# JanEGerken/HEAL-SWIN

Hardware: AMD Instinct MI355X
Metric: images/sec fwd+bwd, HEAL-SWIN nside=256 seg, batch=8 at 1/2/4/8 MI355X (higher is better)
Workload: dtype bf16

## Files before the change

### heal_swin_amd/_lib.py

```python
import ctypes
import os

import numpy as np

_PKG = os.path.dirname(os.path.abspath(__file__))
LIB_PATH = os.path.join(_PKG, "lib", "libhealswin.so")

HS_F32, HS_BF16 = 0, 1
HS_F64 = 3
HS_PRED_LABELS, HS_PRED_ROWS16 = 2, 4
HS_ATTN_COSINE = 1
HS_ATTN_FORCE_VALU = 2
HS_ATTN_RESIDUAL = 4
HS_ATTN_OVERWRITE_GRADS = 8
HS_EPI_BIAS, HS_EPI_GELU, HS_EPI_DGELU, HS_EPI_RESID = 0, 1, 2, 3
HS_ACC_DEFER = 2
HS_MLP_NORM_AFTER = 16
HS_U8, HS_I32, HS_I64 = 8, 9, 10
HS_FLAT_PATCH_ROWS, HS_FLAT_PIXEL_ROWS = 0, 1
HS_DEPTH_L1, HS_DEPTH_L2, HS_DEPTH_HUBER, HS_DEPTH_LOGVAR = 0, 1, 2, 3
HS_DT_NONE, HS_DT_LOG, HS_DT_INV = 0, 1, 2
HS_DT_ZERO_BKG, HS_DT_1000_BKG, HS_DT_AFFINE, HS_DT_INVERSE = 1, 2, 4, 8
HS_DEPTH_STATS_WORDS = 15

c_i64 = ctypes.c_int64
c_int = ctypes.c_int
c_uint = ctypes.c_uint
c_ptr = ctypes.c_void_p
c_float = ctypes.c_float

_SIGNATURES = {
    "hs_nest2ring": [c_int, c_ptr, c_ptr, c_i64],
    "hs_ring2nest": [c_int, c_ptr, c_ptr, c_i64],
    "hs_nest_win_idcs": [c_int, c_ptr],
    "hs_rel_pos_index": [c_int, c_ptr],
    "hs_build_nest_roll_shift": [c_i64, c_int, c_int, c_ptr, c_ptr, c_ptr],
    "hs_build_nest_grid_shift": [c_int, c_int, c_int, c_ptr, c_ptr, c_ptr],
    "hs_build_ring_shift": [c_int, c_int, c_int, c_int, c_ptr, c_ptr, c_ptr],
    "hs_attn_mask_from_labels": [c_ptr, c_i64, c_int, c_ptr],
    "hs_flat_zorder": [c_int, c_int, c_int, c_ptr, c_ptr],
    "hs_build_flat_shift": [c_int, c_int, c_int, c_int, c_int, c_ptr, c_ptr, c_ptr],
    "hs_flat_rel_pos_index": [c_int, c_ptr, c_ptr],
    "hs_flat_attn_mask": [c_int, c_int, c_int, c_int, c_ptr],
    "hs_flat_img_to_rows": [c_ptr, c_int, c_ptr, c_int, c_int, c_int, c_int, c_int, c_int, c_int, c_int, c_i64, c_ptr],
    "hs_flat_rows_to_img": [c_ptr, c_int, c_ptr, c_int, c_int, c_int, c_int, c_int, c_int, c_int, c_int, c_i64, c_ptr],
    "hs_rel_bias_gather": [c_ptr, c_ptr, c_ptr, c_int, c_int, c_int, c_ptr],
    "hs_rel_bias_scatter_grad_sorted_add": [c_ptr, c_ptr, c_ptr, c_ptr, c_int, c_int, c_int, c_ptr],
    "hs_cos_head_scale_fwd": [c_ptr, c_ptr, c_int, c_ptr],
    "hs_cos_head_scale_bwd": [c_ptr, c_ptr, c_ptr, c_int, c_int, c_ptr],
    "hs_rel_bias_gather_many": [c_ptr, c_ptr, c_int, c_ptr, c_ptr, c_int, c_int, c_ptr],
    "hs_rel_bias_scatter_grad_sorted_many": [c_ptr, c_ptr, c_ptr, c_ptr, c_int, c_ptr, c_ptr, c_int, c_int, c_ptr],
    "hs_cos_head_scale_many": [c_ptr, c_ptr, c_ptr, c_ptr, c_ptr, c_int, c_ptr],
# ... 23 lines not shown
    "hs_backproject_labels": [c_ptr, c_int, c_i64, c_i64, c_int, c_i64, c_i64, c_i64, c_ptr, c_i64, c_int, c_ptr, c_ptr],
    "hs_backproject_image": [c_ptr, c_i64, c_i64, c_ptr, c_ptr, c_i64, c_ptr, c_ptr],
    "hs_seg_confusion": [c_ptr, c_int, c_i64, c_i64, c_int, c_i64, c_i64, c_i64, c_ptr, c_i64, c_ptr, c_int, c_ptr, c_ptr, c_ptr],
    "hs_depth_points": [c_ptr, c_int, c_i64, c_i64, c_i64, c_i64, c_i64, c_i64, c_ptr, c_i64, c_ptr, c_int, c_ptr, c_ptr, c_ptr, c_ptr,
                        c_ptr],
    "hs_chamfer_nn": [c_ptr, c_ptr, c_i64, c_i64, c_ptr, c_ptr, c_i64, c_i64, c_i64, c_int, c_ptr, c_ptr, c_ptr, c_ptr, c_ptr, c_ptr,
                      c_ptr],
    "hs_depth_metrics": [c_ptr, c_int, c_i64, c_i64, c_i64, c_i64, c_i64, c_i64, c_i64, c_ptr, c_int, c_i64, c_i64, c_i64, c_int,
                         ctypes.c_double, c_ptr, c_int, c_ptr, c_ptr, c_ptr],
    "hs_backproject_depth": [c_ptr, c_int, c_i64, c_i64, c_i64, c_i64, c_ptr, c_ptr, c_i64, c_ptr, c_ptr],
    "hs_sample_bilinear_u8_f32": [c_ptr, c_int, c_int, c_int, c_int, c_ptr, c_ptr, c_i64, c_ptr, c_ptr],
    "hs_sample_nearest_f32": [c_ptr, c_int, c_int, c_int, c_ptr, c_ptr, c_i64, c_float, c_ptr, c_ptr],
    "hs_depth_target": [c_ptr, c_i64, c_i64, c_ptr, c_i64, c_i64, c_i64, c_i64, c_int, c_int, c_float, c_float, c_ptr],
    "hs_depth_stats_update": [c_ptr, c_i64, c_int, c_int, c_ptr, c_ptr, c_ptr],
    "hs_depth_stats_merge": [c_ptr, c_int, c_ptr, c_ptr],
    "hs_gelu_fwd": [c_ptr, c_ptr, c_i64, ctypes.c_float, ctypes.c_uint64, c_int, c_ptr],
    "hs_gelu_bwd": [c_ptr, c_ptr, c_ptr, c_i64, ctypes.c_float, ctypes.c_uint64, c_int, c_ptr],
    "hs_residual_drop": [c_ptr, c_ptr, c_ptr, c_ptr, c_i64, c_i64, ctypes.c_float, ctypes.c_uint64, c_int, c_ptr],
    "hs_linear_wgrad": [c_ptr, c_ptr, c_ptr, c_ptr, c_ptr, c_i64, c_int, c_int, c_int, c_int, c_ptr],
    "hs_reduce_flush": [c_ptr],
    "hs_set_seed_epoch": [c_ptr],
    "hs_linear_wgrad_gelu": [c_ptr, c_ptr, c_ptr, c_ptr, c_ptr, c_i64, c_int, c_int, c_int, c_int, c_ptr],
    "hs_linear_wgrad_gelu_supported": [c_i64, c_int, c_int, c_int],
    "hs_mlp_fused_supported": [c_int, c_int, c_int],
    "hs_mlp_fused_fwd": [c_ptr, c_ptr, c_ptr, c_ptr, c_ptr, c_ptr, c_ptr, c_ptr, c_ptr, c_ptr, c_ptr, c_ptr, c_ptr, c_i64, c_int, c_int, c_uint,
                         c_int, c_ptr],
    "hs_mlp_fused_bwd": [c_ptr, c_ptr, c_ptr, c_ptr, c_ptr, c_ptr, c_ptr, c_i64, c_int, c_int, c_int, c_ptr],
    "hs_mlp_fused_drop_fwd": [c_ptr, c_ptr, c_ptr, c_ptr, c_ptr, c_ptr, c_ptr, c_ptr, c_ptr, c_ptr, c_ptr, c_ptr, c_ptr, c_ptr, c_i64, c_float,
                              ctypes.c_uint64, ctypes.c_uint64, c_i64, c_int, c_int, c_uint, c_int, c_ptr],
    "hs_mlp_fused_drop_bwd": [c_ptr, c_ptr, c_ptr, c_ptr, c_ptr, c_ptr, c_ptr, c_float, ctypes.c_uint64, c_i64, c_int, c_int, c_int, c_ptr],
    "hs_adam_step": [c_ptr, c_ptr, c_ptr, c_ptr, c_ptr, c_i64, c_float, c_ptr, c_float, c_float, c_float, c_float, c_int, c_ptr, c_ptr],
    "hs_adam_advance": [c_ptr, c_ptr],
    "hs_split_bf16x3": [c_ptr, c_ptr, c_i64, c_int, c_int, c_ptr],
    "hs_gelu_split3": [c_ptr, c_ptr, c_ptr, c_i64, c_int, ctypes.c_float, ctypes.c_uint64, c_ptr],
    "hs_linear_wgrad_ld": [c_ptr, c_i64, c_i64, c_ptr, c_i64, c_i64, c_ptr, c_ptr, c_ptr, c_i64, c_int, c_int, c_int, c_ptr],
    "hs_layernorm_fwd": [c_ptr, c_ptr, c_ptr, c_ptr, c_ptr, c_ptr, c_ptr, c_i64, c_int, c_int, c_ptr],
    "hs_add_layernorm_fwd": [c_ptr, c_ptr, c_ptr, c_ptr, c_ptr, c_ptr, c_ptr, c_ptr, c_i64, c_int, c_int, c_ptr],
    "hs_add_layernorm_bwd": [c_ptr, c_ptr, c_ptr, c_ptr, c_ptr, c_ptr, c_ptr, c_ptr, c_ptr, c_ptr, c_int, c_i64, c_int, c_int, c_ptr],
    "hs_layernorm_drop_fwd": [c_ptr, c_ptr, c_ptr, c_ptr, c_ptr, c_ptr, c_ptr, c_ptr, c_i64, ctypes.c_float, ctypes.c_uint64,
                              c_i64, c_int, c_int, c_ptr],
    "hs_layernorm_drop_bwd": [c_ptr, c_ptr, c_ptr, c_ptr, c_ptr, c_ptr, c_ptr, c_ptr, c_ptr, c_int, c_ptr, c_i64, ctypes.c_float,
                              ctypes.c_uint64, c_i64, c_int, c_int, c_ptr],
    "hs_add_layernorm_drop_fwd": [c_ptr, c_ptr, c_ptr, c_ptr, c_ptr, c_ptr, c_ptr, c_ptr, c_ptr, c_i64, ctypes.c_float,
                                  ctypes.c_uint64, c_i64, c_int, c_int, c_ptr],
    "hs_layernorm_fwd_ex": [c_ptr, c_ptr, c_ptr, c_ptr, c_ptr, c_ptr, c_ptr, c_ptr, c_ptr, c_ptr, c_ptr, c_ptr, c_i64, ctypes.c_float,
                            ctypes.c_uint64, c_i64, c_int, c_int, c_ptr],
# ... 21 lines not shown
    "hs_patch_merge_bwd": [c_ptr, c_ptr, c_ptr, c_ptr, c_ptr, c_ptr, c_ptr, c_ptr, c_ptr, c_ptr, c_ptr, c_ptr, c_ptr, c_int, c_i64,
                           c_int, c_int, c_int, c_ptr],
    "hs_patch_expand_fwd": [c_ptr, c_ptr, c_ptr, c_ptr, c_ptr, c_ptr, c_ptr, c_ptr, c_i64, c_int, c_int, c_int, c_int, c_ptr],
    "hs_patch_expand_bwd": [c_ptr, c_ptr, c_ptr, c_ptr, c_ptr, c_ptr, c_ptr, c_ptr, c_ptr, c_ptr, c_ptr, c_ptr, c_ptr, c_int, c_i64,
                            c_int, c_int, c_int, c_int, c_ptr],
}
_OTHER = {
    "hs_version": ([], ctypes.c_char_p),
    "hs_last_error": ([], ctypes.c_char_p),
    "hs_status_string": ([c_int], ctypes.c_char_p),
    "hs_device_count": ([], c_int),
    "hs_get_reserved_cus": ([], c_int),
    "hs_get_seed_epoch": ([], c_ptr),
    "hs_reduce_pending": ([c_ptr], c_int),
    "hs_layernorm_bwd_workspace": ([c_i64, c_int], c_i64),
    "hs_seg_ce_partials": ([c_i64, c_i64], c_i64),
    "hs_depth_loss_partials": ([c_i64, c_i64], c_i64),
    "hs_depth_points_workspace": ([c_i64, c_i64], c_i64),
    "hs_depth_metrics_partials": ([c_i64], c_i64),
    "hs_depth_stats_partials": ([c_i64], c_i64),
    "hs_ln_head_partials": ([c_i64], c_i64),
    "hs_expand_ln_head_blocks": ([c_i64], c_i64),
    "hs_linear_wgrad_workspace": ([c_i64, c_int, c_int], c_i64),
    "hs_window_attn_bwd_workspace": ([c_int, c_i64, c_int, c_int, c_int, c_int], c_i64),
    "hs_patch_merge_bwd_workspace": ([c_i64, c_int, c_int], c_i64),
    "hs_window_attn_module_bwd_chain_workspace": ([c_int, c_i64, c_int, c_int, c_int], c_i64),
    "hs_patch_expand_bwd_workspace": ([c_i64, c_int, c_int, c_int], c_i64),
}
EXPORTED_SYMBOLS = sorted(list(_SIGNATURES) + list(_OTHER))


def _load():
    if not os.path.exists(LIB_PATH):
        raise RuntimeError(
            f"libhealswin.so not found at {LIB_PATH}: build it first (python heal_swin_amd/build.py, or "
            "__graft_entry__.build()).  heal_swin_amd has no CPU or PyTorch fallback."
        )
    lib = ctypes.CDLL(LIB_PATH)
    for name, argtypes in _SIGNATURES.items():
        fn = getattr(lib, name)
        fn.argtypes = argtypes
        fn.restype = c_int
    for name, (argtypes, restype) in _OTHER.items():
        fn = getattr(lib, name)
        fn.argtypes = argtypes
        fn.restype = restype
# ... 133 lines not shown
```

### heal_swin_amd/csrc/linear_wgrad.hip

```cpp
#include <cstdlib>
#include <type_traits>
#include <utility>

#include "hs_gelu.h"

namespace hs {
namespace {

typedef __attribute__((ext_vector_type(8))) __bf16 bf16x8;
typedef __attribute__((ext_vector_type(16))) float f32x16;
typedef __attribute__((ext_vector_type(4))) short s16x4;
typedef __attribute__((ext_vector_type(8))) short s16x8;
typedef __attribute__((address_space(3))) s16x4 lds_s16x4;

constexpr int kTileK = 128;
constexpr int kTok = 32;
constexpr int kMaxSlices = 2048;
constexpr int kReduceChunks = 32;
__host__ __device__ constexpr int row_stride(int cols) { return cols * 2 + 64; }

template <int LD>
__device__ __forceinline__ bf16x8 tr_frag(const unsigned char* tile, int tok0, int col0, int lane) {
    const int L = lane & 15, nblk = (lane >> 4) & 1;
    const unsigned char* a = tile + (tok0 + (L >> 2)) * LD + (col0 + nblk * 16 + (L & 3) * 4) * 2;
// ... 172 lines not shown
#pragma unroll
            for (int rg = 0; rg < 256 / YCH; ++rg) t += bred[rg * TN + tid];
            if (n0 + tid < n_out) part_b[(int64_t)slice * ((int64_t)n_out * k_in + n_out) + n0 + tid] = t;
        }
    }
}

typedef __attribute__((address_space(3))) void lds_void;
typedef __attribute__((ext_vector_type(4))) unsigned int u32x4;

template <int RB>
__device__ __forceinline__ s16x8 tr_frag_asm(uint32_t a, int ks) {
    s16x4 lo, hi;
    if (ks == 0) {
        asm volatile("ds_read_b64_tr_b16 %0, %1" : "=v"(lo) : "v"(a));
        asm volatile("ds_read_b64_tr_b16 %0, %1 offset:%2" : "=v"(hi) : "v"(a), "n"(4 * RB));
    } else {
        asm volatile("ds_read_b64_tr_b16 %0, %1 offset:%2" : "=v"(lo) : "v"(a), "n"(16 * RB));
        asm volatile("ds_read_b64_tr_b16 %0, %1 offset:%2" : "=v"(hi) : "v"(a), "n"(20 * RB));
    }
    return s16x8{lo[0], lo[1], lo[2], lo[3], hi[0], hi[1], hi[2], hi[3]};
}

template <int NB, int TK, bool GX = false>
__global__ void __launch_bounds__(TK * 2, 2) wgrad_dma_kernel(const uint16_t* __restrict__ dy, const uint16_t* __restrict__ x,
                                                           float* __restrict__ part_w, float* __restrict__ part_b,
                                                           int64_t rows, int n_out, int k_in, Geometry g, int ldy, int ldx, int yc0, int xc0) {
#if defined(__HIP_DEVICE_COMPILE__)
    constexpr int TN = 64 * NB;
    constexpr int WK = TK / 64, NW = 2 * WK, NT = 64 * NW;
    constexpr int YRB = TN * 2, XRB = TK * 2;
    constexpr int YB = kTok * YRB, XB = kTok * XRB;
    constexpr int STAGE = YB + XB, NSTAGE = TK == 256 ? 4 : 3, AH = NSTAGE - 1;
    constexpr int YI = YB / 1024 / NW, XI = XB / 1024 / NW;
    constexpr int YCH = YRB / 16, XCH = XRB / 16;
    __shared__ __attribute__((aligned(16))) unsigned char smem[NSTAGE * STAGE];
    float* bred = (float*)smem;

    const int tid = threadIdx.x, lane = tid & 63, wave = tid >> 6, half = lane >> 5;
    const int wn = wave / WK, wk = wave % WK;
    int slice, tile;
    if (!block_to_work(g, blockIdx.x, slice, tile)) return;
    const int tn = tile / g.tiles_k, tk = tile % g.tiles_k;
    const int n0 = tn * TN, k0 = tk * TK;
    const int64_t m_begin = (int64_t)slice * g.rows_per_slice;
    int64_t m_end = m_begin + g.rows_per_slice;
    if (m_end > rows) m_end = rows;
    const int m_len = m_end > m_begin ? (int)(m_end - m_begin) : 0;
    const int nst = (m_len + kTok - 1) / kTok;
    const bool do_bias = part_b != nullptr && tk == 0;

    const __amdgpu_buffer_rsrc_t rs_y = __builtin_amdgcn_make_buffer_rsrc((void*)(dy + m_begin * ldy), 0, m_len * ldy * 2, 0x00020000);
    const __amdgpu_buffer_rsrc_t rs_x = __builtin_amdgcn_make_buffer_rsrc((void*)(x + m_begin * ldx), 0, m_len * ldx * 2, 0x00020000);
    int voff_y[YI], voff_x[XI];
#pragma unroll
    for (int j = 0; j < YI; ++j) {
        const int p = (wave * YI + j) * 64 + lane, row = p / YCH, pc = p % YCH;
        voff_y[j] = row * ldy * 2 + (yc0 + n0) * 2 + ((pc ^ ((row & 3) << 2)) << 4);
    }
#pragma unroll
    for (int j = 0; j < XI; ++j) {
        const int p = (wave * XI + j) * 64 + lane, row = p / XCH, pc = p % XCH;
        voff_x[j] = row * ldx * 2 + (xc0 + k0) * 2 + ((pc ^ ((row & 3) << 2)) << 4);
    }
    const int ystep = kTok * ldy * 2, xstep = kTok * ldx * 2;
    auto issue = [&](int b) {
// ... 32 lines not shown

    s16x8 af[2][NB], bf[2][2];
    auto read_frags = [&](auto buf_c) {
        constexpr int buf = decltype(buf_c)::value;
#pragma unroll
        for (int ks = 0; ks < 2; ++ks) {
#pragma unroll
            for (int j = 0; j < 2; ++j) bf[ks][j] = tr_frag_asm<XRB>(lds0 + buf * STAGE + xoff[j], ks);
#pragma unroll
            for (int i = 0; i < NB; ++i) af[ks][i] = tr_frag_asm<YRB>(lds0 + buf * STAGE + yoff[i], ks);
        }
    };
    auto wait_half = [&](int ks) {
        if constexpr (NB == 4) {
            if (ks == 0) asm volatile("s_waitcnt lgkmcnt(12)" : "+v"(bf[0][0]), "+v"(bf[0][1]), "+v"(af[0][0]), "+v"(af[0][1]), "+v"(af[0][2]), "+v"(af[0][3]));
            else asm volatile("s_waitcnt lgkmcnt(0)" : "+v"(bf[1][0]), "+v"(bf[1][1]), "+v"(af[1][0]), "+v"(af[1][1]), "+v"(af[1][2]), "+v"(af[1][3]));
        } else {
            if (ks == 0) asm volatile("s_waitcnt lgkmcnt(8)" : "+v"(bf[0][0]), "+v"(bf[0][1]), "+v"(af[0][0]), "+v"(af[0][1]));
            else asm volatile("s_waitcnt lgkmcnt(0)" : "+v"(bf[1][0]), "+v"(bf[1][1]), "+v"(af[1][0]), "+v"(af[1][1]));
        }
    };
    auto mma_half = [&](int ks) {
        if constexpr (GX) {
#pragma unroll
            for (int j = 0; j < 2; ++j) {
                u32x4 w = __builtin_bit_cast(u32x4, bf[ks][j]);
#pragma unroll
                for (int e = 0; e < 4; ++e) {
                    const f32x2 v = gelu2(f32x2{__uint_as_float(w[e] << 16), __uint_as_float(w[e] & 0xffff0000u)});
                    w[e] = pack_bf16x2(v.x, v.y);
                }
                bf[ks][j] = __builtin_bit_cast(s16x8, w);
            }
        }
#pragma unroll
        for (int i = 0; i < NB; ++i)
#pragma unroll
            for (int j = 0; j < 2; ++j)
                acc[i][j] = __builtin_amdgcn_mfma_f32_32x32x16_bf16(__builtin_bit_cast(bf16x8, af[ks][i]), __builtin_bit_cast(bf16x8, bf[ks][j]), acc[i][j], 0, 0, 0);
    };
    auto bias_sums = [&](auto buf_c) {
        constexpr int buf = decltype(buf_c)::value;
        constexpr int PS = kTok / (NT / YCH);
        u32x4 v[PS];
        const uint32_t ba = lds0 + buf * STAGE + boff;
        asm volatile("ds_read_b128 %0, %1" : "=v"(v[0]) : "v"(ba));
        asm volatile("ds_read_b128 %0, %1 offset:%2" : "=v"(v[1]) : "v"(ba), "n"((NT / YCH) * YRB));
        if constexpr (PS == 4) {
            asm volatile("ds_read_b128 %0, %1 offset:%2" : "=v"(v[2]) : "v"(ba), "n"(2 * (NT / YCH) * YRB));
            asm volatile("ds_read_b128 %0, %1 offset:%2" : "=v"(v[3]) : "v"(ba), "n"(3 * (NT / YCH) * YRB));
            asm volatile("s_waitcnt lgkmcnt(0)" : "+v"(v[0]), "+v"(v[1]), "+v"(v[2]), "+v"(v[3]));
        } else {
            asm volatile("s_waitcnt lgkmcnt(0)" : "+v"(v[0]), "+v"(v[1]));
        }
#pragma unroll
// ... 252 lines not shown
            const int kk = k0 + wk * 64 + b2 * 32 + l31;
#pragma unroll
            for (int r = 0; r < 16; ++r) {
                const int nn = n0 + wn * 64 + a * 32 + (r & 3) + 8 * (r >> 2) + 4 * half;
                if (nn < n_out && kk < k_in) dst[(int64_t)nn * k_in + kk] = acc[a][b2][r];
            }
        }
    if (do_bias) {
        __syncthreads();
        const int rg = tid >> 5, c4 = (tid & 31) * 4;
#pragma unroll
        for (int i = 0; i < 4; ++i) bred[rg * TN + c4 + i] = bsum[i];
        __syncthreads();
        if (tid < TN) {
            float t = 0.f;
#pragma unroll
            for (int r2 = 0; r2 < 8; ++r2) t += bred[r2 * TN + tid];
            if (n0 + tid < n_out) part_b[(int64_t)slice * ((int64_t)n_out * k_in + n_out) + n0 + tid] = t;
        }
    }
#endif
}

}
}

extern "C" {

int64_t hs_linear_wgrad_workspace(int64_t rows, int n_out, int k_in) {
    if (rows <= 0 || n_out <= 0 || k_in <= 0) return 0;
    const hs::Geometry g = hs::make_geometry(rows, n_out, k_in), f = hs::make_geometry_f32(rows, n_out, k_in);
    const int64_t a = g.slices + (g.chunks > 1 ? g.chunks : 0), b = f.slices + (f.chunks > 1 ? f.chunks : 0);
    return (a > b ? a : b) * ((int64_t)n_out * k_in + n_out);
}

namespace {
int linear_wgrad_impl(const void* dy, const void* x, float* dw, float* dbias, float* workspace, int64_t rows, int n_out, int k_in,
                      int accumulate, int dtype, void* stream, int ldy, int ldx, int yc0, int xc0, bool gelu_x = false);
}

int hs_linear_wgrad(const void* dy, const void* x, float* dw, float* dbias, float* workspace, int64_t rows, int n_out,
                    int k_in, int accumulate, int dtype, void* stream) {
    return linear_wgrad_impl(dy, x, dw, dbias, workspace, rows, n_out, k_in, accumulate, dtype, stream, n_out, k_in, 0, 0);
}

int hs_linear_wgrad_gelu_supported(int64_t rows, int n_out, int k_in, int dtype) {
// ... 26 lines not shown
    if (dtype == HS_BF16 && (n_out % 4 || k_in % 8))
        return fail(HS_ERR_UNSUPPORTED, "bf16: n_out must be a multiple of 4 and k_in a multiple of 8");
    if (dtype == HS_F32 && (n_out % 4 || k_in % 4)) return fail(HS_ERR_UNSUPPORTED, "fp32: n_out and k_in must be multiples of 4");
    Geometry g = dtype == HS_F32 ? make_geometry_f32(rows, n_out, k_in) : make_geometry(rows, n_out, k_in);
    if (gelu_x && !(dtype == HS_BF16 && g.dma && g.tile_k != 256 && g.tile_n != 256))
        return fail(HS_ERR_UNSUPPORTED, "hs_linear_wgrad_gelu: bf16 and the 128 x 128 LDS-DMA tile only (n_out <= 128-class shapes)");
    const bool strided = ldy != n_out || ldx != k_in || yc0 || xc0;
    if (strided) {
        if (!g.dma || g.rows_per_slice * (int64_t)(ldy > ldx ? ldy : ldx) * 2 >= ((int64_t)1 << 31))
            return fail(HS_ERR_UNSUPPORTED, "hs_linear_wgrad_ld: a token slice exceeds the 2 GiB buffer-offset range");
    }
    if (dtype == HS_BF16 && n_out % 8 && !g.dma) return fail(HS_ERR_UNSUPPORTED, "n_out must be a multiple of 8 for slices beyond 2 GiB");
    if (dtype == HS_F32 && !g.dma) return fail(HS_ERR_UNSUPPORTED, "fp32: a token slice exceeds the 2 GiB buffer-offset range");
    const int64_t n = (int64_t)n_out * k_in, rec = n + n_out;
    float* part_w = workspace;
    float* part_b = dbias ? workspace + n : nullptr;
    hipStream_t s = (hipStream_t)stream;
    const dim3 grid((unsigned)(8 * g.per_xcd));
    const uint16_t* dyp = (const uint16_t*)dy;
    const uint16_t* xp = (const uint16_t*)x;
    if (dtype == HS_F32)
        hipLaunchKernelGGL(wgrad_dma_f32_kernel, grid, dim3(256), 0, s, (const float*)dy, (const float*)x, part_w, part_b, rows, n_out,
                           k_in, g);
    else if (g.dma && g.tile_k == 256)
        hipLaunchKernelGGL((wgrad_dma_kernel<4, 256>), grid, dim3(512), 0, s, dyp, xp, part_w, part_b, rows, n_out, k_in, g, ldy, ldx, yc0, xc0);
    else if (g.dma && g.tile_n == 256)
        hipLaunchKernelGGL((wgrad_dma_kernel<4, 128>), grid, dim3(256), 0, s, dyp, xp, part_w, part_b, rows, n_out, k_in, g, ldy, ldx, yc0, xc0);
    else if (g.dma && gelu_x)
        hipLaunchKernelGGL((wgrad_dma_kernel<2, 128, true>), grid, dim3(256), 0, s, dyp, xp, part_w, part_b, rows, n_out, k_in, g, ldy, ldx, yc0, xc0);
    else if (g.dma)
        hipLaunchKernelGGL((wgrad_dma_kernel<2, 128>), grid, dim3(256), 0, s, dyp, xp, part_w, part_b, rows, n_out, k_in, g, ldy, ldx, yc0, xc0);
    else if (g.tile_n == 256)
        hipLaunchKernelGGL(wgrad_kernel<4>, grid, dim3(256), 0, s, dyp, xp, part_w, part_b, rows, n_out, k_in, g);
    else
        hipLaunchKernelGGL(wgrad_kernel<2>, grid, dim3(256), 0, s, dyp, xp, part_w, part_b, rows, n_out, k_in, g);
    HS_LAUNCH_CHECK("linear_wgrad");
    const int64_t count = dbias ? rec : n;
    if (accumulate & HS_ACC_DEFER)
        return reduce_defer(part_w, rec, g.slices, n, count, dw, dbias, accumulate & 1, s);
    return reduce_now(part_w, rec, g.slices, n, count, dw, dbias, accumulate & 1, s);
}
}

}
```

### heal_swin_amd/ops/gemm.py

```python
import math
import os

import torch

from .. import _lib
from .._lib import check, lib, ptr, stream_ptr
from .runtime import RT, _cast_param, _defer_flag, _defer_keep, _require_gpu, _sink_buffer, _timed


OWN_GEMM = os.environ.get("HS_OWN_GEMM", "auto")


OWN_GELU_MAX_K = 4096
OWN_DGELU_MAX_K = 1024
OWN_BIAS_MAX_K = 0


class GemmTuner:
    MIN_FLOP = 1 << 33

    def __init__(self):
        self.picks = {}
        self.trials = {}

    @staticmethod
    def key(m, n, k):
        return (max(1, int(m)).bit_length(), int(n), int(k))

    def pick(self, m, n, k, device):
# ... 213 lines not shown
def _lib_matmul(dy2, w, res=None):
    m, n = dy2.shape
    if isinstance(dy2, _Split):
        with _timed(_lib_tag("dgrad bf16x3", m, w.shape[1], 3 * n), dy2.device, 4 * (m * n + m * w.shape[1]), 6 * m * n * w.shape[1]):
            return _mm_f32(dy2.t3, _weight_split(w, True).t(), res)
    if _bf16x3_ok(dy2, w.shape[1], n) and w.dtype == torch.float32 and w.shape[1] % 8 == 0:
        with _timed(_lib_tag("dgrad bf16x3", m, w.shape[1], 3 * n), dy2.device, 4 * (m * n + m * w.shape[1]), 6 * m * n * w.shape[1]):
            dx = _mm_f32(split3(dy2, 0), _weight_split(w, True).t(), res)
        return dx
    with _timed(_lib_tag("dgrad", m, w.shape[1], n), dy2.device, 2 * (m * n + m * w.shape[1]), 2 * m * n * w.shape[1]):
        return dy2 @ w if res is None else torch.addmm(res, dy2, w)


def _cast_param_t(p, dtype, cache=None):
    if cache is None:
        cache = RT.cast_cache if RT.cast_cache is not None else RT.last_cast_cache
    c = cache.get_t(p, dtype) if (cache is not None and p.dim() == 2 and cache.current(p)) else None
    if c is None:
        n_out = p.shape[0]
        c = p.detach().to(dtype).view(n_out, -1).t().contiguous()
    return c


def _param_grads(dy2, x2, weight, bias, want_w, want_b, x3=None, gelu_x=False):
    n_out = weight.shape[0]
    k_in = weight.numel() // n_out
    if not (want_w or want_b):
        return None, None
    if x2 is None:
        assert x3 is not None and dy2.dtype == torch.float32
        hip_ok = dy2.is_contiguous() and n_out % 8 == 0
        assert hip_ok
    else:
        hip_ok = (x2.is_contiguous() and dy2.is_contiguous() and n_out % 4 == 0 and
                  ((x2.dtype == torch.bfloat16 and k_in % 8 == 0) or (x2.dtype == torch.float32 and k_in % 4 == 0)))
    wbuf = _sink_buffer(weight) if (hip_ok and want_w) else None
    bbuf = _sink_buffer(bias) if (wbuf is not None and want_b) else None
    if wbuf is not None and (not want_b or bbuf is not None):
        aw = RT.async_wgrad
        wbuf = wbuf.view(n_out, k_in)
        if aw is not None:
            cur = torch.cuda.current_stream(dy2.device)
            aw.stream.wait_stream(cur)
            dy2.record_stream(aw.stream)
            (x2 if x2 is not None else x3).record_stream(aw.stream)
            with torch.cuda.stream(aw.stream):
                LinearFn._wgrad_hip(dy2, x2, n_out, k_in, want_b, wbuf, bbuf, x3, gelu_x)
        else:
            LinearFn._wgrad_hip(dy2, x2, n_out, k_in, want_b, wbuf, bbuf, x3, gelu_x)
        RT.grad_sink.deposited(weight)
        if want_b:
            RT.grad_sink.deposited(bias)
        return None, None
    dw = db = None
    if hip_ok:
        dw32, db32 = LinearFn._wgrad_hip(dy2, x2, n_out, k_in, want_b, x3=x3, gelu_x=gelu_x)
        dw = dw32.to(weight.dtype).view(weight.shape) if want_w else None
        db = db32.to(bias.dtype) if want_b else None
    else:
        assert not gelu_x
        if want_w:
            dw = (dy2.t() @ x2).to(weight.dtype).view(weight.shape)
        if want_b:
            db = dy2.sum(0).to(bias.dtype)
    return dw, db


class LinearFn(torch.autograd.Function):

    @staticmethod
# ... 139 lines not shown
```

### heal_swin_amd/ops/runtime.py

```python
import contextlib
import ctypes
import os
import weakref

import torch

from .. import _lib
from .._lib import check, lib, ptr, stream_ptr


KERNEL_TIMINGS = None
TIMED_PREFIXES = None


class RuntimeState:

    def __init__(self):
        self.grad_sink = None
        self.async_wgrad = None
        self.cast_cache = None
        self.last_cast_cache = None
        self.prefer_own_gemm = False
        self.zero_padded_grads = weakref.WeakValueDictionary()
        self.weight_epoch = 0
# ... 62 lines not shown

def _extras(x, row_scale, drop_p, seed):
    if row_scale is None and not drop_p:
        return None
    rows = x.numel() // x.shape[-1]
    rs, rps = None, 1
    if row_scale is not None:
        rs = row_scale.detach().to(torch.float32).contiguous()
        assert rows % rs.numel() == 0
        rps = rows // rs.numel()
    if drop_p and seed is None:
        seed = _draw_seed()
    return rs, rps, float(drop_p or 0.0), int(seed or 0)


def _sink_buffer(p):
    sink = RT.grad_sink
    return None if (sink is None or p is None) else sink.grad_buffer(p)


DEFER_REDUCTIONS = os.environ.get("HS_DEFER_REDUCE", "1") != "0"
_DEFER_KEEP = {}
_DEFER_FLUSH_AT = 32


def _defer_flag(device):
    sink = RT.grad_sink
    ok = DEFER_REDUCTIONS and sink is not None and RT.async_wgrad is None and getattr(sink, "flushes_reductions", False)
    return _lib.HS_ACC_DEFER if ok else 0


def _defer_keep(device, *workspaces):
    s = torch.cuda.current_stream(device).cuda_stream
    keep = _DEFER_KEEP.setdefault(s, [])
    keep.extend(workspaces)
    if int(lib.hs_reduce_pending(ctypes.c_void_p(s))) >= _DEFER_FLUSH_AT:
        flush_reductions(device)


def flush_reductions(device=None):
    if not torch.cuda.is_available():
        return
    s = torch.cuda.current_stream(device).cuda_stream
    check(lib.hs_reduce_flush(ctypes.c_void_p(s)), "hs_reduce_flush")
    keep = _DEFER_KEEP.get(s)
    if keep:
        keep.clear()


class AsyncWgrad:

    def __init__(self, device):
        self.stream = torch.cuda.Stream(device=device)

    def sync(self):
        cur = torch.cuda.current_stream(self.stream.device)
        cur.wait_stream(self.stream)




class ParamCastCache:

    always_refresh = False

    def __init__(self, params, dtype, shadow_of=None):
# ... 82 lines not shown
```

### include/healswin.h

```cpp
#ifndef HEALSWIN_H
#define HEALSWIN_H

#include <stdint.h>

#ifdef __cplusplus
extern "C" {
#endif

typedef enum {
    HS_OK = 0,
    HS_ERR_INVALID_ARG = 1,
    HS_ERR_UNSUPPORTED = 2,
    HS_ERR_HIP = 3,
    HS_ERR_NOT_PERMUTATION = 4
} hs_status;

typedef enum { HS_F32 = 0, HS_BF16 = 1 } hs_dtype;

#define HS_ATTN_COSINE 1u
#define HS_ATTN_FORCE_VALU 2u
#define HS_ATTN_RESIDUAL 4u
#define HS_ATTN_OVERWRITE_GRADS 8u

const char* hs_version(void);
// ... 108 lines not shown
                  int label_bytes, int64_t ignore_index, int dtype, void* stream);
int hs_seg_ce_bwd(const void* logits, const void* labels, const float* class_weights, const float* scale, void* dlogits,
                  int64_t batch, int64_t npix, int n_classes, int64_t stride_b, int64_t stride_k, int64_t stride_p,
                  int64_t dstride_b, int64_t dstride_k, int64_t dstride_p, int label_bytes, int64_t ignore_index,
                  int dtype, void* stream);

#define HS_DEPTH_L1 0
#define HS_DEPTH_L2 1
#define HS_DEPTH_HUBER 2
#define HS_DEPTH_LOGVAR 3
int64_t hs_depth_loss_partials(int64_t batch, int64_t npix);
int hs_depth_loss_fwd(const void* pred, const float* target, float* partials, int64_t batch, int64_t npix, int channels,
                      int64_t stride_b, int64_t stride_c, int64_t stride_p, int kind, float huber_delta, int dtype, void* stream);
int hs_depth_loss_bwd(const void* pred, const float* target, const float* scale, void* dpred, int64_t batch, int64_t npix, int channels,
                      int64_t stride_b, int64_t stride_c, int64_t stride_p, int64_t dstride_b, int64_t dstride_c, int64_t dstride_p,
                      int kind, float huber_delta, int dtype, void* stream);

int64_t hs_linear_wgrad_workspace(int64_t rows, int n_out, int k_in);
int hs_linear_wgrad(const void* dy, const void* x, float* dw, float* dbias, float* workspace,
                    int64_t rows, int n_out, int k_in, int accumulate, int dtype, void* stream);
int hs_linear_wgrad_gelu_supported(int64_t rows, int n_out, int k_in, int dtype);
int hs_linear_wgrad_gelu(const void* dy, const void* h, float* dw, float* dbias, float* workspace, int64_t rows, int n_out, int k_in,
                         int accumulate, int dtype, void* stream);

#define HS_ACC_DEFER 2
int hs_reduce_pending(void* stream);
int hs_reduce_flush(void* stream);

#define HS_MLP_NORM_AFTER 16u
int hs_mlp_fused_supported(int channels, int hidden, int dtype);
int hs_mlp_fused_fwd(const void* x, const float* ln_gamma, const float* ln_beta, const void* w1, const float* b1, const void* w2,
                     const float* b2, void* n_out, float* mean_out, float* rstd_out, void* h_out, void* act_out, void* out, int64_t rows,
                     int channels, int hidden, unsigned flags, int dtype, void* stream);
int hs_mlp_fused_bwd(const void* dy, const void* h, const void* w2_t, const void* w1_t, const void* dres, void* dh, void* dn, int64_t rows,
                     int channels, int hidden, int dtype, void* stream);
int hs_mlp_fused_drop_fwd(const void* x, const float* ln_gamma, const float* ln_beta, const void* w1, const float* b1, const void* w2,
                          const float* b2, void* m_out, float* mean_out, float* rstd_out, void* h_out, void* act_out, void* out,
                          const float* row_scale, int64_t rows_per_sample, float drop_p, uint64_t seed_hidden, uint64_t seed_out,
                          int64_t rows, int channels, int hidden, unsigned flags, int dtype, void* stream);
int hs_mlp_fused_drop_bwd(const void* dy, const void* h, const void* w2_t, const void* w1_t, const void* dres, void* dh, void* dn,
                          float drop_p, uint64_t seed_hidden, int64_t rows, int channels, int hidden, int dtype, void* stream);

int hs_adam_step(float* p, const float* g, float* m, float* v, void* p_bf16, int64_t n, float lr, const float* lr_dev, float beta1,
                 float beta2, float eps, float weight_decay, int decoupled, const int64_t* step, void* stream);
int hs_adam_advance(int64_t* step, void* stream);

// ... 174 lines not shown
```

Before: 56.39.

## Group consecutive bf16 weight-gradient GEMMs into one grouped DMA kernel launch

New measurement: 57.32 (median of 6 runs). 1.7% higher.

```diff
diff --git a/heal_swin_amd/_lib.py b/heal_swin_amd/_lib.py
--- a/heal_swin_amd/_lib.py
+++ b/heal_swin_amd/_lib.py
@@ -28,6 +28,19 @@
 c_uint = ctypes.c_uint
 c_ptr = ctypes.c_void_p
 c_float = ctypes.c_float
+
+
+class WgradProblem(ctypes.Structure):
+    _fields_ = [("dy", c_ptr), ("x", c_ptr), ("dw", c_ptr), ("dbias", c_ptr), ("n_out", c_int), ("k_in", c_int), ("accumulate", c_int),
+                ("gelu_x", c_int)]
+
+
+def wgrad_problems(members):
+    arr = (WgradProblem * len(members))()
+    for q, (dy, x, dw, db, n_out, k_in, acc, gelu_x) in zip(arr, members):
+        q.dy, q.x, q.dw, q.dbias = dy.data_ptr(), x.data_ptr(), dw.data_ptr(), (None if db is None else db.data_ptr())
+        q.n_out, q.k_in, q.accumulate, q.gelu_x = int(n_out), int(k_in), int(acc), int(bool(gelu_x))
+    return arr
 
 _SIGNATURES = {
     "hs_nest2ring": [c_int, c_ptr, c_ptr, c_i64],
@@ -97,6 +110,8 @@
     "hs_set_seed_epoch": [c_ptr],
     "hs_linear_wgrad_gelu": [c_ptr, c_ptr, c_ptr, c_ptr, c_ptr, c_i64, c_int, c_int, c_int, c_int, c_ptr],
     "hs_linear_wgrad_gelu_supported": [c_i64, c_int, c_int, c_int],
+    "hs_linear_wgrad_group_variant": [c_i64, c_int, c_int, c_int],
+    "hs_linear_wgrad_group": [c_ptr, c_int, c_ptr, c_i64, c_int, c_ptr],
     "hs_mlp_fused_supported": [c_int, c_int, c_int],
     "hs_mlp_fused_fwd": [c_ptr, c_ptr, c_ptr, c_ptr, c_ptr, c_ptr, c_ptr, c_ptr, c_ptr, c_ptr, c_ptr, c_ptr, c_ptr, c_i64, c_int, c_int, c_uint,
                          c_int, c_ptr],
@@ -164,6 +179,7 @@
     "hs_ln_head_partials": ([c_i64], c_i64),
     "hs_expand_ln_head_blocks": ([c_i64], c_i64),
     "hs_linear_wgrad_workspace": ([c_i64, c_int, c_int], c_i64),
+    "hs_linear_wgrad_group_workspace": ([c_ptr, c_int, c_i64, c_int], c_i64),
     "hs_window_attn_bwd_workspace": ([c_int, c_i64, c_int, c_int, c_int, c_int], c_i64),
     "hs_patch_merge_bwd_workspace": ([c_i64, c_int, c_int], c_i64),
     "hs_window_attn_module_bwd_chain_workspace": ([c_int, c_i64, c_int, c_int, c_int], c_i64),
diff --git a/heal_swin_amd/csrc/linear_wgrad.hip b/heal_swin_amd/csrc/linear_wgrad.hip
--- a/heal_swin_amd/csrc/linear_wgrad.hip
+++ b/heal_swin_amd/csrc/linear_wgrad.hip
@@ -218,10 +218,21 @@
     return s16x8{lo[0], lo[1], lo[2], lo[3], hi[0], hi[1], hi[2], hi[3]};
 }
 
+constexpr int kMaxGroup = 4;
+struct Member {
+    const uint16_t* dy;
+    const uint16_t* x;
+    float* part_w;
+    float* part_b;
+    int n_out, k_in, ldy, ldx, yc0, xc0, tiles_k, first_tile, gelu;
+};
+struct MemberTable {
+    int count;
+    Member m[kMaxGroup];
+};
+
 template <int NB, int TK, bool GX = false>
-__global__ void __launch_bounds__(TK * 2, 2) wgrad_dma_kernel(const uint16_t* __restrict__ dy, const uint16_t* __restrict__ x,
-                                                           float* __restrict__ part_w, float* __restrict__ part_b,
-                                                           int64_t rows, int n_out, int k_in, Geometry g, int ldy, int ldx, int yc0, int xc0) {
+__global__ void __launch_bounds__(TK * 2, 2) wgrad_dma_kernel(const MemberTable tb, int64_t rows, Geometry g) {
 #if defined(__HIP_DEVICE_COMPILE__)
     constexpr int TN = 64 * NB;
     constexpr int WK = TK / 64, NW = 2 * WK, NT = 64 * NW;
@@ -237,7 +248,19 @@
     const int wn = wave / WK, wk = wave % WK;
     int slice, tile;
     if (!block_to_work(g, blockIdx.x, slice, tile)) return;
-    const int tn = tile / g.tiles_k, tk = tile % g.tiles_k;
+    int mi = 0;
+#pragma unroll
+    for (int i = 1; i < kMaxGroup; ++i)
+        if (i < tb.count && tile >= tb.m[i].first_tile) mi = i;
+    const Member& mb = tb.m[__builtin_amdgcn_readfirstlane(mi)];
+    const uint16_t* __restrict__ dy = mb.dy;
+    const uint16_t* __restrict__ x = mb.x;
+    float* __restrict__ part_w = mb.part_w;
+    float* __restrict__ part_b = mb.part_b;
+    const int n_out = mb.n_out, k_in = mb.k_in, ldy = mb.ldy, ldx = mb.ldx, yc0 = mb.yc0, xc0 = mb.xc0;
+    [[maybe_unused]] const bool gelu = mb.gelu != 0;
+    tile -= mb.first_tile;
+    const int tn = tile / mb.tiles_k, tk = tile % mb.tiles_k;
     const int n0 = tn * TN, k0 = tk * TK;
     const int64_t m_begin = (int64_t)slice * g.rows_per_slice;
     int64_t m_end = m_begin + g.rows_per_slice;
@@ -316,15 +339,17 @@
     };
     auto mma_half = [&](int ks) {
         if constexpr (GX) {
-#pragma unroll
-            for (int j = 0; j < 2; ++j) {
-                u32x4 w = __builtin_bit_cast(u32x4, bf[ks][j]);
-#pragma unroll
-                for (int e = 0; e < 4; ++e) {
-                    const f32x2 v = gelu2(f32x2{__uint_as_float(w[e] << 16), __uint_as_float(w[e] & 0xffff0000u)});
-                    w[e] = pack_bf16x2(v.x, v.y);
+            if (gelu) {
+#pragma unroll
+                for (int j = 0; j < 2; ++j) {
+                    u32x4 w = __builtin_bit_cast(u32x4, bf[ks][j]);
+#pragma unroll
+                    for (int e = 0; e < 4; ++e) {
+                        const f32x2 v = gelu2(f32x2{__uint_as_float(w[e] << 16), __uint_as_float(w[e] & 0xffff0000u)});
+                        w[e] = pack_bf16x2(v.x, v.y);
+                    }
+                    bf[ks][j] = __builtin_bit_cast(s16x8, w);
                 }
-                bf[ks][j] = __builtin_bit_cast(s16x8, w);
             }
         }
 #pragma unroll
@@ -623,6 +648,71 @@
 #endif
 }
 
+inline int dma_variant(const Geometry& g) { return !g.dma ? 0 : (g.tile_k == 256 ? 1 : (g.tile_n == 256 ? 2 : 3)); }
+
+inline void launch_dma(int variant, bool any_gelu, dim3 grid, hipStream_t s, const MemberTable& tb, int64_t rows, const Geometry& g) {
+    if (variant == 1)
+        hipLaunchKernelGGL((wgrad_dma_kernel<4, 256>), grid, dim3(512), 0, s, tb, rows, g);
+    else if (variant == 2)
+        hipLaunchKernelGGL((wgrad_dma_kernel<4, 128>), grid, dim3(256), 0, s, tb, rows, g);
+    else if (any_gelu)
+        hipLaunchKernelGGL((wgrad_dma_kernel<2, 128, true>), grid, dim3(256), 0, s, tb, rows, g);
+    else
+        hipLaunchKernelGGL((wgrad_dma_kernel<2, 128>), grid, dim3(256), 0, s, tb, rows, g);
+}
+
+struct GroupPlan {
+    bool grouped;
+    int variant, any_gelu;
+    Geometry g;
+    int first_tile[kMaxGroup], tiles_k[kMaxGroup];
+    int64_t offset[kMaxGroup], total;
+};
+
+inline GroupPlan plan_group(const hs_wgrad_problem* p, int count, int64_t rows, int dtype) {
+    GroupPlan pl{};
+    pl.grouped = dtype == HS_BF16 && count > 1;
+    int tiles = 0;
+    for (int i = 0; i < count && pl.grouped; ++i) {
+        if (p[i].n_out <= 0 || p[i].k_in <= 0 || p[i].n_out % 4 || p[i].k_in % 8) pl.grouped = false;
+        if (!pl.grouped) break;
+        const Geometry gi = make_geometry(rows, p[i].n_out, p[i].k_in);
+        const int v = dma_variant(gi);
+        if (i == 0) {
+            pl.variant = v;
+            pl.g = gi;
+        }
+        if (v == 0 || v != pl.variant || (p[i].gelu_x && v != 3)) pl.grouped = false;
+        pl.first_tile[i] = tiles;
+        pl.tiles_k[i] = gi.tiles_k;
+        pl.any_gelu |= p[i].gelu_x ? 1 : 0;
+        tiles += gi.tiles;
+    }
+    if (pl.grouped) {
+        Geometry& g = pl.g;
+        g.tiles = tiles;
+        int64_t want = ((int64_t)usable_cus() * (pl.variant == 1 ? 1 : 2)) / tiles;
+        const int64_t max_by_rows = (rows + 511) / 512;
+        if (want > max_by_rows) want = max_by_rows;
+        if (want > kMaxSlices) want = kMaxSlices;
+        if (want < 1) want = 1;
+        g.slices = (int)want;
+        const int64_t rps = (rows + g.slices - 1) / g.slices;
+        g.rows_per_slice = ((rps + kTok - 1) / kTok) * kTok;
+        g.per_xcd = (g.slices * g.tiles + 7) / 8;
+        for (int i = 0; i < count; ++i)
+            if (g.rows_per_slice * (int64_t)(p[i].n_out > p[i].k_in ? p[i].n_out : p[i].k_in) * 2 >= ((int64_t)1 << 31)) pl.grouped = false;
+    }
+    int64_t off = 0;
+    for (int i = 0; i < count; ++i) {
+        pl.offset[i] = off;
+        off += pl.grouped ? (int64_t)pl.g.slices * ((int64_t)p[i].n_out * p[i].k_in + p[i].n_out)
+                          : hs_linear_wgrad_workspace(rows, p[i].n_out, p[i].k_in);
+    }
+    pl.total = off;
+    return pl;
+}
+
 }
 }
 
@@ -695,15 +785,12 @@
     if (dtype == HS_F32)
         hipLaunchKernelGGL(wgrad_dma_f32_kernel, grid, dim3(256), 0, s, (const float*)dy, (const float*)x, part_w, part_b, rows, n_out,
                            k_in, g);
-    else if (g.dma && g.tile_k == 256)
-        hipLaunchKernelGGL((wgrad_dma_kernel<4, 256>), grid, dim3(512), 0, s, dyp, xp, part_w, part_b, rows, n_out, k_in, g, ldy, ldx, yc0, xc0);
-    else if (g.dma && g.tile_n == 256)
-        hipLaunchKernelGGL((wgrad_dma_kernel<4, 128>), grid, dim3(256), 0, s, dyp, xp, part_w, part_b, rows, n_out, k_in, g, ldy, ldx, yc0, xc0);
-    else if (g.dma && gelu_x)
-        hipLaunchKernelGGL((wgrad_dma_kernel<2, 128, true>), grid, dim3(256), 0, s, dyp, xp, part_w, part_b, rows, n_out, k_in, g, ldy, ldx, yc0, xc0);
-    else if (g.dma)
-        hipLaunchKernelGGL((wgrad_dma_kernel<2, 128>), grid, dim3(256), 0, s, dyp, xp, part_w, part_b, rows, n_out, k_in, g, ldy, ldx, yc0, xc0);
-    else if (g.tile_n == 256)
+    else if (g.dma) {
+        MemberTable tb{};
+        tb.count = 1;
+        tb.m[0] = Member{dyp, xp, part_w, part_b, n_out, k_in, ldy, ldx, yc0, xc0, g.tiles_k, 0, gelu_x ? 1 : 0};
+        launch_dma(dma_variant(g), gelu_x, grid, s, tb, rows, g);
+    } else if (g.tile_n == 256)
         hipLaunchKernelGGL(wgrad_kernel<4>, grid, dim3(256), 0, s, dyp, xp, part_w, part_b, rows, n_out, k_in, g);
     else
         hipLaunchKernelGGL(wgrad_kernel<2>, grid, dim3(256), 0, s, dyp, xp, part_w, part_b, rows, n_out, k_in, g);
@@ -715,4 +802,52 @@
 }
 }
 
-}
+int hs_linear_wgrad_group_variant(int64_t rows, int n_out, int k_in, int dtype) {
+    if (dtype != HS_BF16 || rows <= 0 || n_out <= 0 || k_in <= 0 || n_out % 4 || k_in % 8) return 0;
+    return hs::dma_variant(hs::make_geometry(rows, n_out, k_in));
+}
+
+int64_t hs_linear_wgrad_group_workspace(const hs_wgrad_problem* problems, int count, int64_t rows, int dtype) {
+    if (!problems || count < 1 || count > hs::kMaxGroup || rows <= 0) return 0;
+    return hs::plan_group(problems, count, rows, dtype).total;
+}
+
+int hs_linear_wgrad_group(const hs_wgrad_problem* problems, int count, float* workspace, int64_t rows, int dtype, void* stream) {
+    using namespace hs;
+    HS_CHECK_ARG(problems && workspace, "null pointer");
+    HS_CHECK_ARG(count >= 1 && count <= kMaxGroup, "hs_linear_wgrad_group: 1 to 4 problems");
+    HS_CHECK_ARG(rows > 0, "bad shape");
+    HS_CHECK_ARG(dtype == HS_BF16 || dtype == HS_F32, "dtype must be HS_F32 or HS_BF16");
+    const GroupPlan pl = plan_group(problems, count, rows, dtype);
+    if (!pl.grouped) {
+        for (int i = 0; i < count; ++i) {
+            const hs_wgrad_problem& p = problems[i];
+            if (int st = linear_wgrad_impl(p.dy, p.x, p.dw, p.dbias, workspace + pl.offset[i], rows, p.n_out, p.k_in, p.accumulate, dtype,
+                                           stream, p.n_out, p.k_in, 0, 0, p.gelu_x != 0))
+                return st;
+        }
+        return HS_OK;
+    }
+    MemberTable tb{};
+    tb.count = count;
+    for (int i = 0; i < count; ++i) {
+        const hs_wgrad_problem& p = problems[i];
+        HS_CHECK_ARG(p.dy && p.x && p.dw, "null pointer");
+        float* part = workspace + pl.offset[i];
+        tb.m[i] = Member{(const uint16_t*)p.dy, (const uint16_t*)p.x, part, p.dbias ? part + (int64_t)p.n_out * p.k_in : nullptr,
+                         p.n_out, p.k_in, p.n_out, p.k_in, 0, 0, pl.tiles_k[i], pl.first_tile[i], p.gelu_x ? 1 : 0};
+    }
+    hipStream_t s = (hipStream_t)stream;
+    launch_dma(pl.variant, pl.any_gelu != 0, dim3((unsigned)(8 * pl.g.per_xcd)), s, tb, rows, pl.g);
+    HS_LAUNCH_CHECK("linear_wgrad_group");
+    for (int i = 0; i < count; ++i) {
+        const hs_wgrad_problem& p = problems[i];
+        const int64_t n = (int64_t)p.n_out * p.k_in, rec = n + p.n_out, cnt = p.dbias ? rec : n;
+        const int st = (p.accumulate & HS_ACC_DEFER) ? reduce_defer(tb.m[i].part_w, rec, pl.g.slices, n, cnt, p.dw, p.dbias, p.accumulate & 1, s)
+                                                     : reduce_now(tb.m[i].part_w, rec, pl.g.slices, n, cnt, p.dw, p.dbias, p.accumulate & 1, s);
+        if (st) return st;
+    }
+    return HS_OK;
+}
+
+}
diff --git a/heal_swin_amd/ops/gemm.py b/heal_swin_amd/ops/gemm.py
--- a/heal_swin_amd/ops/gemm.py
+++ b/heal_swin_amd/ops/gemm.py
@@ -5,6 +5,7 @@
 
 from .. import _lib
 from .._lib import check, lib, ptr, stream_ptr
+from . import runtime
 from .runtime import RT, _cast_param, _defer_flag, _defer_keep, _require_gpu, _sink_buffer, _timed
 
 
@@ -264,6 +265,43 @@
     return c
 
 
+def _wgrad_group_ok(dy2, x2, n_out, k_in, want_b, bbuf, x3):
+    return bool(runtime.WGRAD_GROUP and x3 is None and x2 is not None and x2.dtype == torch.bfloat16 and dy2.dtype == torch.bfloat16 and
+                (bbuf is not None or not want_b) and _defer_flag(dy2.device) and
+                lib.hs_linear_wgrad_group_variant(dy2.shape[0], n_out, k_in, _lib.HS_BF16) == 1)
+
+
+def _wgrad_issue(members, dev):
+    rows = members[0][0].shape[0]
+    arr = _lib.wgrad_problems(members)
+    ws = torch.empty(int(lib.hs_linear_wgrad_group_workspace(arr, len(members), rows, _lib.HS_BF16)), dtype=torch.float32, device=dev)
+    with _timed("linear_wgrad" if len(members) == 1 else "linear_wgrad group", dev, sum(2 * rows * (m[4] + m[5]) for m in members),
+                sum(2 * rows * m[4] * m[5] for m in members)):
+        check(lib.hs_linear_wgrad_group(arr, len(members), ptr(ws), rows, _lib.HS_BF16, stream_ptr(dev)), "hs_linear_wgrad_group")
+    _defer_keep(dev, ws)
+
+
+def _wgrad_grouped(member):
+    dev = member[0].device
+    s = torch.cuda.current_stream(dev).cuda_stream
+    parked = runtime._PARKED.pop(s, None)
+    if parked is not None and parked[0].shape[0] == member[0].shape[0]:
+        _wgrad_issue([parked, member], dev)
+        return
+    if parked is not None:
+        _wgrad_issue([parked], dev)
+    runtime._PARKED[s] = member
+
+
+def _wgrad_flush_parked(s, device=None):
+    parked = runtime._PARKED.pop(s, None)
+    if parked is not None:
+        _wgrad_issue([parked], parked[0].device)
+
+
+runtime._PARK_FLUSH[:] = [_wgrad_flush_parked]
+
+
 def _param_grads(dy2, x2, weight, bias, want_w, want_b, x3=None, gelu_x=False):
     n_out = weight.shape[0]
     k_in = weight.numel() // n_out
@@ -288,6 +326,8 @@
             (x2 if x2 is not None else x3).record_stream(aw.stream)
             with torch.cuda.stream(aw.stream):
                 LinearFn._wgrad_hip(dy2, x2, n_out, k_in, want_b, wbuf, bbuf, x3, gelu_x)
+        elif _wgrad_group_ok(dy2, x2, n_out, k_in, want_b, bbuf, x3):
+            _wgrad_grouped((dy2, x2, wbuf, bbuf if want_b else None, n_out, k_in, 1 | _lib.HS_ACC_DEFER, gelu_x))
         else:
             LinearFn._wgrad_hip(dy2, x2, n_out, k_in, want_b, wbuf, bbuf, x3, gelu_x)
         RT.grad_sink.deposited(weight)
diff --git a/heal_swin_amd/ops/runtime.py b/heal_swin_amd/ops/runtime.py
--- a/heal_swin_amd/ops/runtime.py
+++ b/heal_swin_amd/ops/runtime.py
@@ -108,6 +108,9 @@
 DEFER_REDUCTIONS = os.environ.get("HS_DEFER_REDUCE", "1") != "0"
 _DEFER_KEEP = {}
 _DEFER_FLUSH_AT = 32
+WGRAD_GROUP = os.environ.get("HS_WGRAD_GROUP", "1") != "0"
+_PARKED = {}
+_PARK_FLUSH = []
 
 
 def _defer_flag(device):
@@ -128,6 +131,8 @@
     if not torch.cuda.is_available():
         return
     s = torch.cuda.current_stream(device).cuda_stream
+    if s in _PARKED:
+        _PARK_FLUSH[0](s, device)
     check(lib.hs_reduce_flush(ctypes.c_void_p(s)), "hs_reduce_flush")
     keep = _DEFER_KEEP.get(s)
     if keep:
diff --git a/include/healswin.h b/include/healswin.h
--- a/include/healswin.h
+++ b/include/healswin.h
@@ -154,6 +154,16 @@
 int hs_linear_wgrad_gelu_supported(int64_t rows, int n_out, int k_in, int dtype);
 int hs_linear_wgrad_gelu(const void* dy, const void* h, float* dw, float* dbias, float* workspace, int64_t rows, int n_out, int k_in,
                          int accumulate, int dtype, void* stream);
+typedef struct hs_wgrad_problem {
+    const void* dy;
+    const void* x;
+    float* dw;
+    float* dbias;
+    int n_out, k_in, accumulate, gelu_x;
+} hs_wgrad_problem;
+int hs_linear_wgrad_group_variant(int64_t rows, int n_out, int k_in, int dtype);
+int64_t hs_linear_wgrad_group_workspace(const hs_wgrad_problem* problems, int count, int64_t rows, int dtype);
+int hs_linear_wgrad_group(const hs_wgrad_problem* problems, int count, float* workspace, int64_t rows, int dtype, void* stream);
 
 #define HS_ACC_DEFER 2
 int hs_reduce_pending(void* stream);
```
